# Orange-OpenSource/Cool-Chic

Measured on AMD Instinct MI355X. Metric: decoded Mpixel/s, higher is better.
Workload: dtype int64+f64 entropy / f32 synthesis; 1 GPU; kodak24; frames_on_rank0=24, frame=512x768 RGB 8-bit, HOP decoder

## Files before the change

### cool_chic_amd/csrc/ccd_entropy_pipe.hip

```cpp
#include <hip/hip_runtime.h>
#include <type_traits>

#include "ccd_device.hpp"
#include "ccd_kernels.hpp"
#include "ccd_laplace.hpp"

namespace ccd {

#if defined(CCD_PIPE_PROFILE) && CCD_PIPE_PROFILE >= 3
#define PROF_T() __builtin_amdgcn_s_memtime()
#define PROF_ADD(var, t0) var += __builtin_amdgcn_s_memtime() - (t0)
#define PROF_SUB(var, t0) var -= __builtin_amdgcn_s_memtime() - (t0)
#else
#define PROF_T() 0ull
#define PROF_ADD(var, t0) (void)(t0)
#define PROF_SUB(var, t0) (void)(t0)
#endif
#if defined(CCD_PIPE_PROFILE) && CCD_PIPE_PROFILE == 2 && defined(CCD_PIPE_TRACE)
#define LPROF_T(cond) __builtin_amdgcn_s_memtime()
#elif defined(CCD_PIPE_PROFILE) && CCD_PIPE_PROFILE == 2
#define LPROF_T(cond) ((cond) ? __builtin_amdgcn_s_memtime() : 0ull)
#else
#define LPROF_T(cond) 0ull
#endif
// ... 942 lines not shown
        int64_t acc = C.s_b[(n_layers - 1) * dim + 2 + o];
        const int32_t* w = C.s_w + C.n_w_hidden + 2 * in_pad + o * in_pad;
#pragma unroll 1
        for (int k = 0; k < dim; ++k) acc += static_cast<int64_t>(ain[k]) * w[k];
        stab[o] = acc;
    }
#pragma unroll 1
    for (int l = 0; l < n_layers - 1; ++l) {
#pragma unroll 1
        for (int o = 0; o < dim; ++o) {
            int64_t acc = C.s_b[l * dim + o];
            const int32_t* w = C.s_w + l * dim * in_pad + o * in_pad;
#pragma unroll 1
            for (int k = 0; k < dim; ++k) acc += static_cast<int64_t>(ain[k]) * w[k];
            aout[o] = static_cast<int32_t>((acc < 0 ? 0 : acc) >> 16);
        }
        int32_t* t = ain; ain = aout; aout = t;
    }
#pragma unroll
    for (int o = 0; o < 2; ++o) {
        int64_t acc = C.s_b[(n_layers - 1) * dim + o] + stab[o];
        const int32_t* w = C.s_w + C.n_w_hidden + o * in_pad;
#pragma unroll 1
        for (int k = 0; k < dim; ++k) acc += static_cast<int64_t>(ain[k]) * w[k];
        if (o == 0) out_mu = acc; else out_ls = acc;
    }
}

constexpr int16_t kFeatSentinel = -32768;

struct ExactArgs {
    const EntropyParams* P;
    uint32_t s_w, s_b, s_ring;
    int n_w_hidden, dim, n_layers, n_sp, in_pad;
    int W, fin, fw, feat_plane, ring_mask, fstride;
};
struct ExactOut { int64_t mu, ls; };
__device__ __forceinline__ ExactOut exact_pixel(const ExactArgs& A, int y, int x) {
    const EntropyParams& P = *A.P;
    const int lane = threadIdx.x & 63;
    const int dim = A.dim, n_layers = A.n_layers, n_sp = A.n_sp, in_pad = A.in_pad;
    const int32_t* s_w = reinterpret_cast<const int32_t*>(ccd_pipe_smem + A.s_w);
    const int64_t* s_b = reinterpret_cast<const int64_t*>(ccd_pipe_smem + A.s_b);
    const int8_t* s_ring = reinterpret_cast<const int8_t*>(ccd_pipe_smem + A.s_ring);
    uint64_t xin = 0;
    if (lane < dim) {
        int64_t v = 0;
        if (lane < n_sp) {
            const int yy = y - P.ctx_dy[lane], xx = x + P.ctx_dx[lane];
            if (yy >= 0 && xx >= 0 && xx < A.W) v = s_ring[(yy & A.ring_mask) * 64 + ((xx + 10 * yy) & 63)];
        } else if (A.fin > 0) {
            const int pos = (y >> 1) * A.fw + (x >> 1);
            v = reinterpret_cast<const int16_t*>(P.ifce_feat)[pos * A.fstride + (lane - n_sp)];
            if (v == kFeatSentinel) v = static_cast<int64_t>(static_cast<float>(P.ifce_wide[(lane - n_sp) * A.feat_plane + pos]));
        }
        xin = static_cast<uint64_t>(v) << 16;
    }
    auto bcast = [&](uint64_t v, int k) {
        const uint32_t lo = static_cast<uint32_t>(__shfl(static_cast<int>(static_cast<uint32_t>(v)), k));
        const uint32_t hi = static_cast<uint32_t>(__shfl(static_cast<int>(static_cast<uint32_t>(v >> 32)), k));
        return (static_cast<uint64_t>(hi) << 32) | lo;
    };
    auto layer = [&](const int32_t* wt, const int64_t* bias, int n_out, uint64_t xv) {
        const int o = min(lane, n_out - 1);
        uint64_t acc = static_cast<uint64_t>(bias[o]);
#pragma unroll 1
        for (int k = 0; k < dim; ++k) acc += bcast(xv, k) * static_cast<uint64_t>(static_cast<int64_t>(wt[o * in_pad + k]));
        return acc;
    };
    const uint64_t stab = layer(s_w + A.n_w_hidden + 2 * in_pad, s_b + (n_layers - 1) * dim + 2, 2, xin);
    uint64_t xv = xin;
#pragma unroll 1
    for (int l = 0; l < n_layers - 1; ++l) {
        const int64_t a = static_cast<int64_t>(layer(s_w + l * dim * in_pad, s_b + l * dim, dim, xv));
        xv = static_cast<uint64_t>((a < 0 ? 0 : a) >> 16);
    }
    const uint64_t out = layer(s_w + A.n_w_hidden, s_b + (n_layers - 1) * dim, 2, xv) + stab;
    ExactOut r;
    r.mu = static_cast<int64_t>(bcast(out, 0));
    r.ls = static_cast<int64_t>(bcast(out, 1));
    return r;
}

template <int NV, int kLpp, bool MF, bool DYN_RING, bool DYN, class SH>
__device__ __forceinline__ uint32_t producer_grid(const PipeCtx& C_run, unsigned long long* prof, const GridSeg& seg) {
    constexpr int in_pad = 4 * NV;
    static_assert(!SH::fixed || (!MF && SH::dim <= in_pad && SH::dim > in_pad - 4 && SH::n_sp >= 1 && SH::n_layers >= 2), "ShapeFix: vector-ALU path, matching width");
    PipeCtx C_fix = C_run;
    if constexpr (SH::fixed) {
        constexpr PipeLayout L = pipe_layout(SH::dim, SH::n_layers, in_pad, kRingRows, 0);
        C_fix.s_ring.off = L.ring; C_fix.s_w.off = L.w; C_fix.s_b.off = L.b; C_fix.s_act.off = L.act; C_fix.s_a.off = L.a; C_fix.s_tab.off = L.tab;
        C_fix.s_meta.off = L.meta; C_fix.s_rcp.off = L.rcp; C_fix.s_exp.off = L.exp; C_fix.s_ready.off = L.ready; C_fix.s_consumed.off = L.consumed;
        C_fix.s_abort.off = L.abort; C_fix.n_w_hidden = L.n_w_hidden; C_fix.ring_mask = kRingRows - 1;
#if defined(CCD_PIPE_TRACE)
        C_fix.trace_off = L.end;
#endif
        C_fix.dim = SH::dim; C_fix.n_layers = SH::n_layers; C_fix.n_sp = SH::n_sp; C_fix.k_left = 0;
    }
    const PipeCtx& C = C_fix;
    constexpr int kTaskPix = 64 / kLpp;
    constexpr int kBpx = kTaskPix == 2 ? 8 : 16;
    constexpr int kHalves = kBpx / kTaskPix;
    constexpr int kNSlots = kRows / kBpx;
    constexpr int NOUT = (in_pad + kLpp - 1) / kLpp;
    const int lane = threadIdx.x & 63;
    const int pw = uni(static_cast<int>(threadIdx.x >> 6) - 1);
    const EntropyParams& P = *C.P;
    const int dim = SH::fixed ? SH::dim : uni(C.dim), n_layers = SH::fixed ? SH::n_layers : uni(C.n_layers), n_sp = SH::fixed ? SH::n_sp : uni(C.n_sp);
    const int W = uni(C.W);
    const int k_left = SH::fixed ? 0 : uni(C.k_left), fin = uni(C.fin), fw = uni(C.fw);
    const uint32_t seq_base = uni(C.seq_base);
    int32_t* act = C.s_act + pw * ((DYN_RING ? 16 : 8) * in_pad + 4);
    int32_t* const act_dummy = act + (DYN_RING ? 16 : 8) * in_pad;
    (void)act_dummy;
    const int px = MF ? (lane & 15) : lane / kLpp;
    const int q = MF ? (lane >> 4) : lane % kLpp;
    const int ring_mask = DYN_RING ? uni(C.ring_mask) : kRingRows - 1, n_if = uni(C.n_if), mf_bits = uni(P.mfma);
    (void)n_if; (void)mf_bits;
    const int4* act_row = reinterpret_cast<const int4*>(act + px * in_pad);
    unsigned long long lt_prev_end = 0;
    (void)lt_prev_end;
    int ctx_dy_l[NOUT], ctx_dx_l[NOUT];
#pragma unroll
    for (int t = 0; t < NOUT; ++t) {
        const int k = q + kLpp * t;
        ctx_dy_l[t] = k < n_sp ? P.ctx_dy[k] : 0;
        ctx_dx_l[t] = k < n_sp ? P.ctx_dx[k] : 0;
    }
    const glb_ptr<const int16_t> ifce_feat = (glb_ptr<const int16_t>)reinterpret_cast<const int16_t*>(P.ifce_feat);
    const int feat_plane = uni(C.fh) * fw;
    const int fstride = SH::fixed ? feat_stride(SH::dim - SH::n_sp) : uni(C.fstride);
    int32_t mf_dxy[8], mf_wl[7];
    if constexpr (MF) {
#pragma unroll
        for (int t = 0; t < 8; ++t) {
            const int k = q + 4 * t;
            mf_dxy[t] = k < n_sp ? static_cast<int32_t>((static_cast<uint32_t>(P.ctx_dy[k]) << 16) | (static_cast<uint32_t>(P.ctx_dx[k]) & 0xffffu)) : 0;
        }
#pragma unroll
        for (int r = 0; r < 7; ++r) {
            const int o = r < 4 ? 4 * q + r : 16 + q;
            int32_t w = 0;
            if (k_left >= 0) {
                if (r < 5) w = o < dim ? C.s_w[o * in_pad + k_left] : 0;
                else w = C.s_w[C.n_w_hidden + 2 * in_pad + (r - 5) * in_pad + k_left];
            }
            mf_wl[r] = w;
        }
    }
    (void)mf_dxy; (void)mf_wl;
    constexpr uint32_t kTaskShift = kTaskPix == 8 ? 3 : (kTaskPix == 4 ? 2 : 1), kBpxShift = kBpx == 32 ? 5 : (kBpx == 16 ? 4 : 3), kHalvesShift = kBpxShift - kTaskShift;
    StepWalk it;
    it.init(static_cast<uint32_t>(uni(C.H)), static_cast<uint32_t>(W));
    uint32_t seq = seq_base;
    uint32_t pix0 = uni(C.px_base), prev_pix0 = pix0, prev2_pix0 = pix0, prev_moved = 0;
    const uint32_t seg_first = uni(seg.first), seg_steps = uni(seg.steps);
    const bool seg_body = uni(seg.body ? 1 : 0) != 0;
    if (seg_first > 0u) {
        it.seek_before(seg_first);
        pix0 += uni(seg.pix_before);
        prev_pix0 = pix0 - it.n;
        prev2_pix0 = prev_pix0 - (seg_first > 1u ? it.len_of(seg_first - 2u) : 0u);
        prev_moved = it.moved;
    }
    uint32_t phase = static_cast<uint32_t>((static_cast<unsigned long long>(seq_base) * kHalves) % kProducers);
    const bool split = k_left >= 0 && W > 9 && n_layers >= 2;
    const uint32_t n_steps_total = it.W <= 9u ? it.H * it.W : it.W + 10u * (it.H - 1u);
    const uint32_t seg_end = seg_first + seg_steps;
    const auto walk_on = [&]() {
        prev2_pix0 = prev_pix0; prev_pix0 = pix0; pix0 += it.n; prev_moved = it.moved;
        const uint32_t nx = it.x0 + 1u, mv = nx == it.W ? 1u : 0u;
        it.x0 = mv ? it.W - 10u : nx; it.y0 += mv; it.moved = mv; --it.left;
        it.n = min(it.H - it.y0, ((it.x0 * 0xcccdu) >> 19) + 1u);
    };
    while (n_steps_total - it.left < seg_end && it.next()) {
        const uint32_t seg_n = seg_body ? uni(seg.n_pix) : it.n;
        const uint32_t seg_pix0 = pix0;
        const uint32_t nb = (seg_n + kBpx - 1) >> kBpxShift;
        const uint32_t n_tasks = (seg_n + kTaskPix - 1) >> kTaskShift;
        const uint32_t seq0 = seq;
        uint32_t t_first = static_cast<uint32_t>(pw) - phase;
        t_first += static_cast<int32_t>(t_first) < 0 ? kProducers : 0;
        {
            for (uint32_t task = t_first; task < n_tasks; task += kProducers) {
                const uint32_t j = task >> kHalvesShift;
                const int half = static_cast<int>(task & (kHalves - 1));
                seq = seq0 + j;
                const int slot = static_cast<int>(seq & (kNSlots - 1));
                const int i0 = static_cast<int>(task << kTaskShift);
                const int cnt = min(kTaskPix, static_cast<int>(seg_n) - i0);
                while (seg_pix0 + static_cast<uint32_t>(i0) >= pix0 + it.n) walk_on();
                const uint32_t ia = seg_pix0 + static_cast<uint32_t>(i0) - pix0;
                const uint32_t n_a = min(static_cast<uint32_t>(cnt), it.n - ia);
                const uint32_t bx1 = it.x0 + 1u, b_moved = bx1 == static_cast<uint32_t>(W) ? 1u : 0u;
                const uint32_t bx0 = b_moved ? static_cast<uint32_t>(W) - 10u : bx1, by0 = it.y0 + b_moved;
                const bool in_b = static_cast<uint32_t>(px) >= n_a;
                const int ii = in_b ? px - static_cast<int>(n_a) : static_cast<int>(ia) + px;
                const int y = static_cast<int>(in_b ? by0 : it.y0) + ii, x = static_cast<int>(in_b ? bx0 : it.x0) - 10 * ii;
                const uint32_t dy1 = it.moved, dy2 = it.moved + prev_moved;
                const uint32_t prev_n = pix0 - prev_pix0, prev2_n = prev_pix0 - prev2_pix0;
                uint32_t f_raw[NOUT];
                bool f_has[NOUT];
                if constexpr (!MF) {
                    const int fo = (y >> 1) * fw + (x >> 1);
#pragma unroll
                    for (int t = 0; t < NOUT; ++t) {
                        const int k = q + kLpp * t;
                        f_has[t] = fin > 0 && px < cnt && k >= n_sp && k < dim;
                        f_raw[t] = reinterpret_cast<glb_ptr<const uint16_t>>(ifce_feat)[f_has[t] ? fo * fstride + (k - n_sp) : 0];
                    }
                } else {
#pragma unroll
                    for (int t = 0; t < NOUT; ++t) { f_raw[t] = 0; f_has[t] = false; }
                }
                unsigned long long bad_lanes = 0ull;
                const uint32_t need_slot = seq >= static_cast<uint32_t>(kNSlots) ? seq - kNSlots + 1 : 0;
                const bool ends_in_b = n_a < static_cast<uint32_t>(cnt);
                const uint32_t last1 = ends_in_b ? static_cast<uint32_t>(cnt) - n_a : ia + static_cast<uint32_t>(cnt);
                const uint32_t need_px = ends_in_b ? pix0 + min(last1 + b_moved, it.n) : prev_pix0 + min(last1 + dy1, prev_n);
                const uint32_t need_early_px = ends_in_b ? prev_pix0 + min(last1 + b_moved + dy1, prev_n)
                                                         : prev2_pix0 + min(last1 + dy2, prev2_n);
                unsigned long long lt_a = 0, lt_b = 0, lt_c = 0, lt_d = 0;
                (void)lt_a; (void)lt_b; (void)lt_c; (void)lt_d;
                unsigned narrow_mask = 0;
                constexpr int kPasses = (kTaskPix + 3) / 4;
                uint32_t win_mu[kPasses] = {}, win_rcp[kPasses] = {}, win_ent[kPasses] = {}, win_top[kPasses] = {};
                uint32_t win_left_m = 0, win_keep_m = 0, win_e0 = 0, win_e1 = 0;
                (void)win_mu; (void)win_rcp; (void)win_ent; (void)win_top; (void)win_left_m; (void)win_keep_m; (void)win_e0; (void)win_e1;
                unsigned long long wide_lanes = 0ull;
                RowMeta& meta = *C.s_meta;
                if constexpr (MF) {
                    const int n = px, g = q;
                    const bool live = n < cnt;
                    int32_t f0 = 0, f1 = 0;
                    if (live && fin > 0) {
                        const int fo = (y >> 1) * fw + (x >> 1);
                        if (g < n_if) f0 = ifce_feat[fo * fstride + g];
                        if (g + 4 < n_if) f1 = ifce_feat[fo * fstride + g + 4];
                    }
                    lt_a = LPROF_T(pw == 0);
#if defined(CCD_PIPE_PROFILE) && CCD_PIPE_PROFILE == 2
                    if (pw == 0 && lt_prev_end) prof[4] += lt_a - lt_prev_end;
#endif
                    {
                        const unsigned long long t0 = PROF_T();
                        if (!wait_ge2(C.s_consumed, need_slot, split ? need_early_px : need_px, C.s_abort)) return seq;
                        PROF_ADD(prof[0], t0);
                    }
                    lt_b = LPROF_T(pw == 0);
                    const unsigned long long t_g = PROF_T();
                    {
                        const int mi = (g == 0 && live) ? slot * kBpx + half * kTaskPix + n : kRows;
                        meta.cell[mi] = static_cast<uint32_t>(((y & ring_mask) << 6) | ((x + 10 * y) & 63));
                        meta.goff[mi] = static_cast<uint32_t>(y * W + x);
                    }
                    uint32_t w0 = 0, w1 = 0;
#pragma unroll
                    for (int t = 0; t < 8; ++t) {
                        if (4 * t < n_sp) {
                            const int k = g + 4 * t;
                            const int yy = y - (mf_dxy[t] >> 16), xx = x + static_cast<int16_t>(mf_dxy[t] & 0xffff);
                            const bool take = live && k < n_sp && yy >= 0 && xx >= 0 && xx < W && !(split && k == k_left);
                            const int cell = take ? (yy & ring_mask) * 64 + ((xx + 10 * yy) & 63) : 0;
                            int32_t v = C.s_ring[cell];
                            v = take ? v : 0;
                            if (t < 4) w0 |= static_cast<uint32_t>(v & 0xff) << (8 * t);
                            else w1 |= static_cast<uint32_t>(v & 0xff) << (8 * (t - 4));
                        }
                    }
                    const uint32_t d0 = (static_cast<uint32_t>(f0) + 0x8080u) ^ 0x8080u, d1 = (static_cast<uint32_t>(f1) + 0x8080u) ^ 0x8080u;
                    const i32x4 bop = {static_cast<int>(w0), static_cast<int>(w1), static_cast<int>((d0 & 0xffffu) | (d1 << 16)), 0};
                    PROF_ADD(prof[1], t_g);
                    const unsigned long long t_m = PROF_T();
                    const i32x4* sa = reinterpret_cast<const i32x4*>(static_cast<uint32_t*>(C.s_a)) + lane;
                    const i32x4 zero4 = {0, 0, 0, 0};
                    int64_t pre[5], st0, st1;
                    {
                        i32x4 c1[2][4];
#pragma unroll
                        for (int t = 0; t < 2; ++t)
#pragma unroll
                            for (int s = 0; s < 4; ++s) c1[t][s] = __builtin_amdgcn_mfma_i32_16x16x64_i8(sa[(t * 4 + s) * 64], bop, zero4, 0, 0, 0);
                        const int64_t* bl = C.s_b;
#pragma unroll
                        for (int r = 0; r < 4; ++r) {
                            const int o = 4 * g + r;
                            const int64_t bias = bl[min(o, dim - 1)];
                            pre[r] = mf_comb4(c1[0], r, o < dim ? bias : 0);
                        }
                        {
                            const int64_t bias = bl[min(16 + g, dim - 1)];
                            pre[4] = mf_comb4(c1[1], 0, 16 + g < dim ? bias : 0);
                        }
                        st0 = mf_comb4(c1[1], 1, bl[(n_layers - 1) * dim + 2]);
                        st1 = mf_comb4(c1[1], 2, bl[(n_layers - 1) * dim + 3]);
                    }
                    const i32x4* sl_out = sa + (kMfLayer1 + (n_layers - 2) * kMfHidden) * 64;
                    i32x4 a_h[10], a_o[5];
                    int64_t b_h[5];
                    if (n_layers > 2) {
#pragma unroll
                        for (int s = 0; s < 10; ++s) a_h[s] = sa[(kMfLayer1 + s) * 64];
#pragma unroll
                        for (int r = 0; r < 5; ++r) {
                            const int o = r < 4 ? 4 * g + r : 16 + g;
                            const int64_t bias = C.s_b[dim + min(o, dim - 1)];
                            b_h[r] = o < dim ? bias : 0;
                        }
                    }
#pragma unroll
                    for (int s = 0; s < 5; ++s) a_o[s] = sl_out[s * 64];
// ... 8 lines not shown
                        PROF_SUB(prof[2], t0);
                        PROF_ADD(prof[5], t0);
                        if (live && x >= 1) xleft = static_cast<int32_t>(C.s_ring[(y & ring_mask) * 64 + ((x - 1 + 10 * y) & 63)]) << 16;
                    }
                    lt_d = LPROF_T(pw == 0);
                    const unsigned long long t_h = PROF_T();
                    int32_t av[5];
                    uint32_t big = 0;
#pragma unroll
                    for (int r = 0; r < 5; ++r) {
                        mad64(pre[r], xleft, mf_wl[r]);
                        const int64_t a = pre[r] < 0 ? 0 : pre[r];
                        av[r] = static_cast<int32_t>(a >> 16);
                        big |= static_cast<uint32_t>(av[r]);
                    }
                    mad64(st0, xleft, mf_wl[5]);
                    mad64(st1, xleft, mf_wl[6]);
                    for (int l = 1; l < n_layers - 1; ++l) {
                        const i32x4 b2 = mf_pack15(av);
                        i32x4 c2[5], c2b[5];
#pragma unroll
                        for (int s = 0; s < 5; ++s) c2[s] = __builtin_amdgcn_mfma_i32_16x16x64_i8(a_h[s], b2, zero4, 0, 0, 0);
                        if (dim > 16) {
#pragma unroll
                            for (int s = 0; s < 5; ++s) c2b[s] = __builtin_amdgcn_mfma_i32_16x16x64_i8(a_h[5 + s], b2, zero4, 0, 0, 0);
                        }
#pragma unroll
                        for (int r = 0; r < 4; ++r) {
                            const int64_t a = mf_comb5(c2, r, b_h[r]);
                            av[r] = static_cast<int32_t>((a < 0 ? 0 : a) >> 16);
                            big |= static_cast<uint32_t>(av[r]);
                        }
                        av[4] = 0;
                        if (dim > 16) {
                            const int64_t a = mf_comb5(c2b, 0, b_h[4]);
                            av[4] = static_cast<int32_t>((a < 0 ? 0 : a) >> 16);
                            big |= static_cast<uint32_t>(av[4]);
                        }
                        if (l + 1 < n_layers - 1) {
                            const i32x4* sl = sa + (kMfLayer1 + l * kMfHidden) * 64;
#pragma unroll
                            for (int s = 0; s < 10; ++s) a_h[s] = sl[s * 64];
#pragma unroll
                            for (int r = 0; r < 5; ++r) {
                                const int o = r < 4 ? 4 * g + r : 16 + g;
                                const int64_t bias = C.s_b[(l + 1) * dim + min(o, dim - 1)];
                                b_h[r] = o < dim ? bias : 0;
                            }
                        }
                    }
                    PROF_ADD(prof[6], t_h);
                    const unsigned long long t_o = PROF_T();
                    int64_t out_mu, out_ls;
                    {
                        const i32x4 b3 = mf_pack15(av);
                        i32x4 c3[5];
#pragma unroll
                        for (int s = 0; s < 5; ++s) c3[s] = __builtin_amdgcn_mfma_i32_16x16x64_i8(a_o[s], b3, zero4, 0, 0, 0);
                        out_mu = mf_comb5(c3, 0, b_mu) + st0;
                        out_ls = mf_comb5(c3, 1, b_ls) + st1;
                    }
                    if (__ballot((big >> mf_bits) != 0u) != 0ull) {
                        if (g == 0 && live) mf_exact_task<NV>(C, act, n, y, x, W, fin, fw, feat_plane, ring_mask, out_mu, out_ls);
                    }
                    const int64_t m8 = (out_mu >> 24) + kMuOffset, s8 = (out_ls >> 24) + kScaleOffset;
                    const int32_t idx_mu = static_cast<int32_t>(m8 < 0 ? 0 : (m8 > kNumMu - 1 ? kNumMu - 1 : m8));
                    const int32_t idx_sc = static_cast<int32_t>(s8 < 0 ? 0 : (s8 > kNumScale - 1 ? kNumScale - 1 : s8));
                    const int mpx = slot * kBpx + half * kTaskPix + n;
                    if (g == 0 && live) {
                        meta.mu_idx[mpx] = idx_mu;
                        meta.rcp[mpx] = C.s_rcp[idx_sc];
                    }
                    narrow_mask = static_cast<unsigned>(__ballot(g == 0 && live && idx_sc <= kNarrowMaxScale)) & 0xffffu;
                    PROF_ADD(prof[2], t_m);
                    PROF_ADD(prof[7], t_o);
#if defined(CCD_PIPE_PROFILE) && CCD_PIPE_PROFILE >= 3
                    prof[8] += 1;
#endif
                } else {
                lt_a = LPROF_T(pw == 0);
#if defined(CCD_PIPE_PROFILE) && CCD_PIPE_PROFILE == 2
                if (pw == 0 && lt_prev_end) prof[4] += lt_a - lt_prev_end;
#endif
                {
                    const unsigned long long t0 = PROF_T();
                    if (!wait_ge2(C.s_consumed, need_slot, split ? need_early_px : need_px, C.s_abort)) return seq;
                    PROF_ADD(prof[0], t0);
                }
                lt_b = LPROF_T(pw == 0);
                const unsigned long long t_g = PROF_T();
                {
                    const int mi = (q == 0 && px < cnt) ? slot * kBpx + half * kTaskPix + px : kRows;
                    meta.cell[mi] = static_cast<uint32_t>(((y & ring_mask) << 6) | ((x + 10 * y) & 63));
                    meta.goff[mi] = static_cast<uint32_t>(y * W + x);
                }
                {
                    typedef unsigned int u32x4 __attribute__((ext_vector_type(4)));
                    const u32x4 z4 = {0u, 0u, 0u, 0u};
                    uint2* const tab0 = C.s_tab + static_cast<size_t>(slot * kBpx + half * kTaskPix) * 64;
#pragma unroll
                    for (int j = 0; j < (kTaskPix * 24 + 63) / 64; ++j) {
                        const int t = lane + 64 * j, row = t / 24, e2 = t - 24 * row;
                        uint2* const dst = row < cnt ? &tab0[row * 64 + 16 + 2 * e2] : C.s_tab + kRows * 64 + 16 + 2 * (e2 % 24);
                        *reinterpret_cast<u32x4*>(dst) = z4;
                    }
                }
                {
                    int32_t rr[NOUT];
#pragma unroll
                    for (int t = 0; t < NOUT; ++t) {
                        const int yy = y - ctx_dy_l[t], xx = x + ctx_dx_l[t];
                        rr[t] = C.s_ring[(yy & ring_mask) * 64 + ((xx + 10 * yy) & 63)];
                    }
                    if constexpr (NOUT == 1) asm volatile("" : "+v"(rr[0]));
                    else if constexpr (NOUT == 2) asm volatile("" : "+v"(rr[0]), "+v"(rr[1]));
                    else if constexpr (NOUT == 3) asm volatile("" : "+v"(rr[0]), "+v"(rr[1]), "+v"(rr[2]));
                    else if constexpr (NOUT == 4) asm volatile("" : "+v"(rr[0]), "+v"(rr[1]), "+v"(rr[2]), "+v"(rr[3]));
                    else {
#pragma unroll
                        for (int t = 0; t < NOUT; ++t) asm volatile("" : "+v"(rr[t]));
                    }
                    int32_t fv[NOUT];
                    bool feat_bad = false;
#pragma unroll
                    for (int t = 0; t < NOUT; ++t) {
                        asm volatile("" : "+v"(f_raw[t]));
                        fv[t] = f_has[t] ? static_cast<int32_t>(static_cast<int16_t>(f_raw[t])) : 0;
                        feat_bad |= DYN && fv[t] == kFeatSentinel;
                    }
                    if constexpr (DYN) bad_lanes = __ballot(feat_bad);
#pragma unroll
                    for (int t = 0; t < NOUT; ++t) {
                        const int k = q + kLpp * t;
                        const int yy = y - ctx_dy_l[t], xx = x + ctx_dx_l[t];
                        const int32_t v = k < n_sp ? ((yy >= 0 && xx >= 0 && xx < W && !(split && k == k_left)) ? rr[t] : 0) : fv[t];
                        int32_t* const dst = k < in_pad ? act + px * in_pad + k : act_dummy;
                        *dst = v << 16;
                    }
                }
                PROF_ADD(prof[1], t_g);
                const unsigned long long t_m = PROF_T();
                int4 xv[NV];
#pragma unroll
                for (int v = 0; v < NV; ++v) xv[v] = act_row[v];
                PROF_ADD(prof[4], t_m);
                const unsigned long long t_s = PROF_T();
                int64_t so[2];
                const int qs = q < 2 ? q : 1;
                {
                    const int4* wr = reinterpret_cast<const int4*>(C.s_w + C.n_w_hidden + 2 * in_pad + qs * in_pad);
                    so[0] = C.s_b[(n_layers - 1) * dim + 2 + qs];
                    so[1] = 0;
                    int4 wv[NV];
#pragma unroll
                    for (int v = 0; v < NV; ++v) wv[v] = wr[v];
#pragma unroll
                    for (int v = 0; v < NV; ++v) {
                        const int4 w = wv[v];
                        mad64(so[0], xv[v].x, w.x); mad64(so[1], xv[v].y, w.y); mad64(so[0], xv[v].z, w.z); mad64(so[1], xv[v].w, w.w);
                    }
                }
                PROF_ADD(prof[5], t_s);
                const unsigned long long t_h = PROF_T();
                int64_t acc0[NOUT], acc0_b = 0;
                (void)acc0_b;
                int32_t wleft[NOUT], wleft_stab = 0;
                if (n_layers >= 2) {
                    const int32_t* wl = C.s_w;
                    const int64_t* bl = C.s_b;
                    const int4* wr[NOUT];
                    const int kl = split ? k_left : 0;
#pragma unroll
                    for (int t = 0; t < NOUT; ++t) {
                        const int oc = min(q + kLpp * t, dim - 1);
                        wr[t] = reinterpret_cast<const int4*>(wl + oc * in_pad);
                        acc0[t] = bl[oc];
                        wleft[t] = wl[oc * in_pad + kl];
                    }
                    wleft_stab = C.s_w[C.n_w_hidden + 2 * in_pad + qs * in_pad + kl];
                    int4 w[NOUT], wn[NOUT];
#pragma unroll
                    for (int t = 0; t < NOUT; ++t) w[t] = wr[t][0];
#pragma unroll
                    for (int v = 0; v < NV; ++v) {
                        if (v + 1 < NV) {
#pragma unroll
                            for (int t = 0; t < NOUT; ++t) wn[t] = wr[t][v + 1];
                        }
                        if constexpr (NOUT == 1) { CCD_MAD4_PAIR(acc0, acc0_b, xv[v], w) } else { CCD_MAD4(acc0, xv[v], w, NOUT) }
#pragma unroll
                        for (int t = 0; t < NOUT; ++t) w[t] = wn[t];
                    }
                    if constexpr (NOUT == 1) acc0[0] += acc0_b;
                }
                int32_t xleft = 0;
                const int mpx = slot * kBpx + half * kTaskPix + px;
                uint32_t mu_dst = lds_addr(&meta.mu_idx[px < cnt && q == 0 ? mpx : kRows]);
                uint32_t rcp_dst = lds_addr(&meta.rcp[px < cnt && q == 1 ? mpx : kRows]);
                int32_t rcp_lanes = q == 1 ? -1 : 0, wide_above = px < cnt && q == 1 ? kNarrowMaxScale : 0x7fffffff;
                asm volatile("" : "+v"(mu_dst), "+v"(rcp_dst), "+v"(rcp_lanes), "+v"(wide_above));
#pragma unroll
                for (int k = 0; k < kPasses; ++k) {
                    const int u = lane >> 4, e = lane & 15;
                    const int mine = 4 * k + u;
                    const bool valid = mine < cnt;
                    const int mi = slot * kBpx + half * kTaskPix + (valid ? mine : 4 * k);
                    win_mu[k] = lds_addr(&meta.mu_idx[mi]);
                    win_rcp[k] = lds_addr(&meta.rcp[mi]);
                    win_ent[k] = lds_addr(&C.s_tab[static_cast<size_t>(valid ? mi : kRows) * 64 + e]);
                    win_top[k] = lds_addr(&meta.top[valid && e == 0 ? mi : kRows]);
                    asm volatile("" : "+v"(win_mu[k]), "+v"(win_rcp[k]), "+v"(win_ent[k]), "+v"(win_top[k]));
                }
                win_left_m = (lane & 15) == 15 ? 0u : ~0u;
                win_keep_m = ((lane & 15) == 0 || (lane & 15) == 15) ? 0u : ~0u;
                win_e0 = (lane & 15) == 0 ? (1u << kRcPrecision) - 1u : 0u;
                win_e1 = (lane & 15) == 1 ? 1u : 0u;
                asm volatile("" : "+v"(win_left_m), "+v"(win_keep_m), "+v"(win_e0), "+v"(win_e1));
                lt_c = LPROF_T(pw == 0);
                if (split) {
                    const unsigned long long t0 = PROF_T();
                    const uint32_t want = uni(need_px);
                    const uint32_t cell = static_cast<uint32_t>((y & ring_mask) * 64 + ((x - 1 + 10 * y) & 63));
                    uint32_t seen_v;
                    int32_t r;
                    asm volatile("ds_read_b32 %0, %2 offset:4\n\tds_read_i8 %1, %3\n\ts_waitcnt lgkmcnt(0)"
                                 : "=&v"(seen_v), "=&v"(r) : "v"(C.s_consumed.off), "v"(C.s_ring.off + cell) : "memory");
                    if (__builtin_expect(static_cast<int32_t>(uni(seen_v) - want) < 0, 0)) {
                        unsigned spins = 0;
                        do {
                            if ((++spins & 1023u) == 0) {
                                if (lds_load_acquire(C.s_abort) != 0) return seq;
                                if (spins > kSpinLimit) { lds_write_release(C.s_abort, static_cast<uint32_t>(-CCD_ERR_HIP)); return seq; }
                            }
                            asm volatile("ds_read_b32 %0, %2 offset:4\n\tds_read_i8 %1, %3\n\ts_waitcnt lgkmcnt(0)"
                                         : "=&v"(seen_v), "=&v"(r) : "v"(C.s_consumed.off), "v"(C.s_ring.off + cell) : "memory");
                        } while (static_cast<int32_t>(uni(seen_v) - want) < 0);
                    }
                    PROF_ADD(prof[0], t0);
                    PROF_SUB(prof[2], t0);
                    PROF_SUB(prof[6], t0);
                    xleft = (px < cnt && x >= 1) ? r << 16 : 0;
                }
                lt_d = LPROF_T(pw == 0);
                __builtin_amdgcn_s_setprio(1);
                mad64(so[0], xleft, wleft_stab);
                const int64_t stab = so[0] + so[1];
                if (n_layers >= 2) {
#pragma unroll
                    for (int t = 0; t < NOUT; ++t) {
                        mad64(acc0[t], xleft, wleft[t]);
                        const int o = q + kLpp * t;
                        int32_t* const dst = o < dim ? act + px * in_pad + o : act_dummy;
                        *dst = relu_q16(acc0[t]);
                    }
#pragma unroll
                    for (int v = 0; v < NV; ++v) xv[v] = act_row[v];
                }
                for (int l = 1; l < n_layers - 1; ++l) {
                    const int32_t* wl = C.s_w + l * dim * in_pad;
                    const int64_t* bl = C.s_b + l * dim;
                    int64_t acc[NOUT], acc_b = 0;
                    (void)acc_b;
                    const int4* wr[NOUT];
#pragma unroll
                    for (int t = 0; t < NOUT; ++t) {
                        const int oc = min(q + kLpp * t, dim - 1);
                        wr[t] = reinterpret_cast<const int4*>(wl + oc * in_pad);
                        acc[t] = bl[oc];
                    }
                    int4 w[NOUT], wn[NOUT];
#pragma unroll
                    for (int t = 0; t < NOUT; ++t) w[t] = wr[t][0];
#pragma unroll
                    for (int v = 0; v < NV; ++v) {
                        if (v + 1 < NV) {
#pragma unroll
                            for (int t = 0; t < NOUT; ++t) wn[t] = wr[t][v + 1];
                        }
                        if constexpr (NOUT == 1) { CCD_MAD4_PAIR_SEQ(acc, acc_b, xv[v], w) } else { CCD_MAD4_SEQ(acc, xv[v], w, NOUT) }
#pragma unroll
                        for (int t = 0; t < NOUT; ++t) w[t] = wn[t];
                    }
                    if constexpr (NOUT == 1) acc[0] += acc_b;
#pragma unroll
                    for (int t = 0; t < NOUT; ++t) {
                        const int o = q + kLpp * t;
                        int32_t* const dst = o < dim ? act + px * in_pad + o : act_dummy;
                        *dst = relu_q16(acc[t]);
                    }
#pragma unroll
                    for (int v = 0; v < NV; ++v) xv[v] = act_row[v];
                }
                PROF_ADD(prof[6], t_h);
                const unsigned long long t_o = PROF_T();
                int32_t idx = 0;
                {
                    const int4* wr = reinterpret_cast<const int4*>(C.s_w + C.n_w_hidden + qs * in_pad);
                    int64_t ao[4] = {C.s_b[(n_layers - 1) * dim + qs] + stab, 0, 0, 0};
                    int4 wv[NV];
#pragma unroll
                    for (int v = 0; v < NV; ++v) wv[v] = wr[v];
#pragma unroll
                    for (int v = 0; v < NV; ++v) { CCD_MAD4_QUAD_SEQ(ao, xv[v], wv[v]) }
                    const int64_t acc = (ao[0] + ao[1]) + (ao[2] + ao[3]);
                    const int64_t q8 = acc >> 24;
                    const int64_t off = q8 + (q == 0 ? kMuOffset : kScaleOffset);
                    const int64_t hi = q == 0 ? kNumMu - 1 : kNumScale - 1;
                    idx = static_cast<int32_t>(off < 0 ? 0 : (off > hi ? hi : off));
                    *lds_at<int32_t>(mu_dst) = idx;
                    *lds_at<double>(rcp_dst) = C.s_rcp[idx & rcp_lanes];
                }
                if (DYN && __builtin_expect(bad_lanes != 0ull, 0)) {
                    int n_redo = 0;
                    for (int p = 0; p < cnt; ++p) {
                        if (((bad_lanes >> (p * kLpp)) & ((1ull << kLpp) - 1ull)) == 0ull) continue;
                        ExactArgs A;
                        A.P = C.P; A.s_w = uni(C.s_w.off); A.s_b = uni(C.s_b.off); A.s_ring = uni(C.s_ring.off);
                        A.n_w_hidden = uni(C.n_w_hidden); A.dim = dim; A.n_layers = n_layers; A.n_sp = n_sp; A.in_pad = in_pad;
                        A.W = W; A.fin = fin; A.fw = fw; A.feat_plane = feat_plane; A.ring_mask = ring_mask; A.fstride = fstride;
                        asm volatile("" : "+s"(A.P), "+s"(A.s_w), "+s"(A.s_b), "+s"(A.s_ring), "+s"(A.n_w_hidden), "+s"(A.dim), "+s"(A.n_layers));
                        asm volatile("" : "+s"(A.n_sp), "+s"(A.W), "+s"(A.fin), "+s"(A.fw), "+s"(A.feat_plane), "+s"(A.ring_mask), "+s"(A.fstride));
                        const ExactOut r = exact_pixel(A, __builtin_amdgcn_readlane(y, MF ? p : p * kLpp), __builtin_amdgcn_readlane(x, MF ? p : p * kLpp));
                        if (px == p && q < 2) {
                            const int64_t off = ((q == 0 ? r.mu : r.ls) >> 24) + (q == 0 ? kMuOffset : kScaleOffset);
                            const int64_t hi = q == 0 ? kNumMu - 1 : kNumScale - 1;
                            idx = static_cast<int32_t>(off < 0 ? 0 : (off > hi ? hi : off));
                            if (q == 0) {
                                meta.mu_idx[mpx] = idx;
                            } else {
                                    meta.rcp[mpx] = C.s_rcp[idx];
                            }
                        }
                        ++n_redo;
                    }
                    if (lane == 0) atomicAdd(reinterpret_cast<int*>(P.status) + 39, n_redo);
                }
                wide_lanes = __ballot(idx > wide_above);
                PROF_ADD(prof[2], t_m);
                PROF_ADD(prof[7], t_o);
#if defined(CCD_PIPE_PROFILE) && CCD_PIPE_PROFILE >= 3
                prof[8] += 1;
#endif
                }
                const unsigned long long t_t = PROF_T();
                const int base = slot * kBpx + half * kTaskPix;
                uint2* tab = C.s_tab + static_cast<size_t>(base) * 64;
                if constexpr (!MF) {
#pragma unroll
                    for (int k = 0; k < kPasses; ++k) {
                        if (k > 0 && 4 * k >= cnt) break;
                        const int e = lane & 15;
                        const int mu_idx = *lds_at<int32_t>(win_mu[k]);
                        const double rcp256 = window_rcp256(*lds_at<double>(win_rcp[k]));
                        int top = ((mu_idx + 128) >> 8) - 64 + 6;
                        top = max(kAcLo + 13, min(kAcLo + kAlphabet - 1, top));
                        const int ssym = top - (e - 1);
                        const uint32_t lo_m = static_cast<uint32_t>((kAcLo - ssym) >> 31) & win_left_m;
                        const bool at_top = top == kAcLo + kAlphabet - 1;
                        const uint32_t hi_f = at_top ? win_e0 : 0u, to_full = at_top ? win_e1 : 0u;
                        uint32_t left = window_cum_d256(window_d256(mu_idx, ssym), rcp256, C.s_exp) + static_cast<uint32_t>(ssym - kAcLo);
                        left = (min(left, (1u << kRcPrecision) - 1u) | hi_f) & lo_m;
                        const uint32_t right = static_cast<uint32_t>(__builtin_amdgcn_update_dpp(0, static_cast<int>(left), 0x111, 0xf, 0xf, false));
                        uint2 ent;
                        ent.x = left;
                        ent.y = (right - left + to_full) & win_keep_m;
                        typedef unsigned int u32x2 __attribute__((ext_vector_type(2)));
                        const u32x2 ent2 = {ent.x, ent.y};
                        *lds_at<u32x2>(win_ent[k]) = ent2;
                        *lds_at<int32_t>(win_top[k]) = top;
                    }
                }
                unsigned rest = MF ? narrow_mask : 0u;
                while (rest) {
                    int pix[4];
                    int n_here = 0;
#pragma unroll
                    for (int u = 0; u < 4; ++u) {
                        pix[u] = rest ? __builtin_ctz(rest) : -1;
                        if (rest) { rest &= rest - 1; ++n_here; }
                    }
                    const int u = lane >> 4, e = lane & 15;
                    const int mine = u == 0 ? pix[0] : (u == 1 ? pix[1] : (u == 2 ? pix[2] : pix[3]));
                    const int mi = base + (mine < 0 ? pix[0] : mine);
                    const int mu_idx = meta.mu_idx[mi];
                    int top = ((mu_idx + 128) >> 8) - 64 + 6;
                    top = max(kAcLo + 13, min(kAcLo + kAlphabet - 1, top));
                    const double mu = -64.0 + static_cast<double>(mu_idx) * (1.0 / 256.0);
                    const int ssym = top - (e - 1);
                    uint32_t left = min(window_left(mu, meta.rcp[mi], ssym, C.s_exp), (1u << kRcPrecision) - 1u);
                    left = e == 15 ? 0u : left;
                    const uint32_t right = static_cast<uint32_t>(__builtin_amdgcn_update_dpp(0, static_cast<int>(left), 0x111, 0xf, 0xf, false));
                    uint2 ent;
                    ent.x = left;
                    ent.y = (e == 0 || e == 15) ? 0u : ((e == 1 && ssym == kAcLo + kAlphabet - 1) ? (1u << kRcPrecision) - left : right - left);
                    if (mine >= 0) {
                        tab[mine * 64 + e] = ent;
                        if (e == 0) meta.top[mi] = top;
                    }
                    if constexpr (MF) {
                        typedef unsigned int u32x4 __attribute__((ext_vector_type(4)));
                        const u32x4 z4 = {0u, 0u, 0u, 0u};
#pragma unroll
                        for (int j = 0; j < 2; ++j) {
                            const int t = lane + 64 * j;
                            const int ru = t >= 72 ? 3 : (t >= 48 ? 2 : (t >= 24 ? 1 : 0));
                            const int rp = ru == 0 ? pix[0] : (ru == 1 ? pix[1] : (ru == 2 ? pix[2] : pix[3]));
                            if (t < 96 && rp >= 0) *reinterpret_cast<u32x4*>(&tab[rp * 64 + 16 + 2 * (t - 24 * ru)]) = z4;
                        }
                    }
                    (void)n_here;
                }
                unsigned long long wide = MF ? static_cast<unsigned long long>(((1u << cnt) - 1u) & ~narrow_mask) : wide_lanes;
                while (wide) {
                    const int bit = __builtin_ctzll(wide);
                    wide &= wide - 1;
                    const int i = MF ? bit : bit / kLpp;
                    const int mi = base + i;
                    const int mu_idx = meta.mu_idx[mi];
                    int top = ((mu_idx + 128) >> 8) - 64 + 30;
                    top = max(kAcLo + 61, min(kAcLo + kAlphabet - 1, top));
                    const int ssym = top - (lane - 1);
                    uint32_t left = min(window_left_d256(window_d256(mu_idx, ssym), window_rcp256(meta.rcp[mi]), ssym, C.s_exp), (1u << kRcPrecision) - 1u);
                    left = lane == 63 ? 0u : left;
                    const uint32_t right = __shfl_up(left, 1);
                    uint2 ent;
                    ent.x = left;
                    ent.y = (lane == 0 || lane == 63) ? 0u
                            : ((lane == 1 && ssym == kAcLo + kAlphabet - 1) ? (1u << kRcPrecision) - left : right - left);
                    tab[i * 64 + lane] = ent;
                    if (lane == 0) meta.top[mi] = top;
                }
                asm volatile("" ::: "memory");
                if (lane == 0) __hip_atomic_fetch_or(&C.s_ready[slot], 1u << half, __ATOMIC_RELAXED, __HIP_MEMORY_SCOPE_WORKGROUP);
                __builtin_amdgcn_s_setprio(0);
                asm volatile("" ::: "memory");
                PROF_ADD(prof[3], t_t);
#if defined(CCD_PIPE_PROFILE) && CCD_PIPE_PROFILE == 2
#if defined(CCD_PIPE_TRACE)
                {
                    const unsigned long long lt_e = __builtin_amdgcn_s_memtime();
                    const uint32_t gidx = seq0 * kHalves + task;
                    if (lane == 0 && static_cast<uint32_t>(W) == uni(g_trace_cfg[0]) && uni(g_trace_cfg[1]) - it.left < 64u) {
                        typedef unsigned int u32x4 __attribute__((ext_vector_type(4)));
                                                u32x4* r = reinterpret_cast<u32x4*>(ccd_pipe_smem + C.trace_off + (gidx % kTraceTasks) * 32u);
                        const u32x4 r0 = {(it.left << 12) | ((task & 15u) << 8) | (static_cast<uint32_t>(pw) << 4) | static_cast<uint32_t>(cnt), static_cast<uint32_t>(lt_a),
                                          static_cast<uint32_t>(lt_b), static_cast<uint32_t>(lt_c)};
                        const u32x4 r1 = {static_cast<uint32_t>(lt_d), static_cast<uint32_t>(lt_e), need_px - pix0, static_cast<uint32_t>(lt_a >> 32)};
                        r[0] = r0; r[1] = r1;
                    }
                }
#endif
                if (pw == 0) {
                    const unsigned long long lt_e = __builtin_amdgcn_s_memtime();
                    prof[0] += lt_b - lt_a; prof[1] += lt_c - lt_b; prof[2] += lt_d - lt_c; prof[3] += lt_e - lt_d; prof[8] += 1;
                    lt_prev_end = lt_e;
                }
#endif
            }
        }
        seq = seq0 + nb;
        phase = (phase + nb * kHalves) % kProducers;
        if (seg_body) {
            while (n_steps_total - it.left < seg_end) walk_on();
        }
        prev2_pix0 = prev_pix0;
        prev_pix0 = pix0;
        pix0 += it.n;
        prev_moved = it.moved;
    }
    return seq;
}

template <int NV, bool MF, bool DYN, class SH>
__global__ __launch_bounds__(kPipeThreads) void entropy_pipe_kernel(const EntropyParams* slots_desc) {
    const EntropyParams& P = slots_desc[blockIdx.x];
    const int tid = threadIdx.x;
    const int lane = tid & 63;
    const int wave = __builtin_amdgcn_readfirstlane(tid >> 6);
    const int dim = P.dim;
    constexpr int in_pad = 4 * NV;
    const int n_layers = P.n_layers;
    const int n_if = P.has_ifce ? P.n_ifce_out : 0;

    PipeCtx C;
    C.P = &P;
    const int ring_rows = MF ? P.ring_rows : kRingRows;
    {
        const PipeLayout L = pipe_layout(dim, n_layers, in_pad, ring_rows, MF ? mf_tables(n_layers) : 0);
        C.s_ring.off = L.ring; C.s_w.off = L.w; C.s_b.off = L.b; C.s_act.off = L.act; C.s_a.off = L.a; C.s_tab.off = L.tab;
        C.s_meta.off = L.meta; C.s_rcp.off = L.rcp; C.s_exp.off = L.exp; C.s_ready.off = L.ready; C.s_consumed.off = L.consumed;
        C.s_abort.off = L.abort; C.n_w_hidden = L.n_w_hidden;
#if defined(CCD_PIPE_TRACE)
        C.trace_off = L.end;
#endif
    }
    C.ring_mask = ring_rows - 1;
    constexpr int kActRows = MF ? 16 : 8;
    double* s_rcp = smem_at<double>(C.s_rcp.off);
    double* s_exp = smem_at<double>(C.s_exp.off);
    for (int i = tid; i < kNumScale; i += kPipeThreads) s_rcp[i] = P.rcp_table[i];
    for (int i = tid; i < kExpN; i += kPipeThreads) s_exp[i] = kExpTab[i];
    C.dim = dim; C.n_layers = n_layers; C.n_sp = P.n_spatial; C.n_if = n_if;
    C.fstride = feat_stride(n_if);
    C.k_left = -1;
    for (int k = 0; k < P.n_spatial; ++k) if (P.ctx_dy[k] == 0 && P.ctx_dx[k] == -1) C.k_left = k;

    {
        const int64_t* src = P.arm;
        for (int l = 0; l < n_layers; ++l) {
            const int n_out = (l == n_layers - 1) ? 2 : dim;
            int32_t* wt = C.s_w + (l < n_layers - 1 ? l * dim * in_pad : C.n_w_hidden);
            for (int i = tid; i < n_out * in_pad; i += kPipeThreads) {
                const int o = i / in_pad, k = i - o * in_pad;
                wt[i] = k < dim ? static_cast<int32_t>(src[k * n_out + o]) : 0;
            }
            int64_t* bb = C.s_b + (l < n_layers - 1 ? l * dim : (n_layers - 1) * dim);
// ... 371 lines not shown
```

Baseline: 265.4 Mpixel/s.

## Fuse output layer into per-lane partial sums with DPP reduction and per-pixel table build

The entropy producer's last MLP layer no longer writes the final hidden activations to LDS and re-reads a full row per output lane. Each lane now multiplies its own hidden outputs by the output weights and the partial sums are combined with 64-bit DPP lane reductions. The window/probability table is built by each pixel's own lane group instead of in extra cross-pixel passes that re-read mu/rcp from LDS. The ready-flag atomic is issued through inline asm with exec forced to a single lane. This cuts LDS round-trips and serial passes, but adds fragile DPP/exec inline assembly and depends on specific RowMeta layout assumptions.

```diff
diff --git a/cool_chic_amd/csrc/ccd_entropy_pipe.hip b/cool_chic_amd/csrc/ccd_entropy_pipe.hip
--- a/cool_chic_amd/csrc/ccd_entropy_pipe.hip
+++ b/cool_chic_amd/csrc/ccd_entropy_pipe.hip
@@ -1048,6 +1048,38 @@
     return r;
 }
 
+template <int CTRL>
+__device__ __forceinline__ int64_t dpp_add64(int64_t v) {
+    const uint32_t lo = static_cast<uint32_t>(__builtin_amdgcn_mov_dpp(static_cast<int>(v), CTRL, 0xf, 0xf, true));
+    const uint32_t hi = static_cast<uint32_t>(__builtin_amdgcn_mov_dpp(static_cast<int>(v >> 32), CTRL, 0xf, 0xf, true));
+    typedef unsigned int u32x2 __attribute__((ext_vector_type(2)));
+    const u32x2 other = {lo, hi};
+    return v + __builtin_bit_cast(int64_t, other);
+}
+__device__ __forceinline__ int64_t dpp_add64_row_below(int64_t v) {
+    const uint32_t lo = static_cast<uint32_t>(__builtin_amdgcn_update_dpp(0, static_cast<int>(v), 0x142, 0xa, 0xf, false));
+    const uint32_t hi = static_cast<uint32_t>(__builtin_amdgcn_update_dpp(0, static_cast<int>(v >> 32), 0x142, 0xa, 0xf, false));
+    typedef unsigned int u32x2 __attribute__((ext_vector_type(2)));
+    const u32x2 other = {lo, hi};
+    return v + __builtin_bit_cast(int64_t, other);
+}
+template <int LANES>
+__device__ __forceinline__ void group_sum2(int64_t& a, int64_t& b) {
+    static_assert(LANES == 8 || LANES == 16 || LANES == 32, "a pixel's lane group: part of a DPP row, a row, or two rows");
+    a = dpp_add64<0xB1>(a); b = dpp_add64<0xB1>(b);
+    a = dpp_add64<0x4E>(a); b = dpp_add64<0x4E>(b);
+    a = dpp_add64<0x141>(a); b = dpp_add64<0x141>(b);
+    if constexpr (LANES >= 16) { a = dpp_add64<0x140>(a); b = dpp_add64<0x140>(b); }
+    if constexpr (LANES == 32) { a = dpp_add64_row_below(a); b = dpp_add64_row_below(b); }
+}
+__device__ __forceinline__ int32_t table_index(int64_t sum, int32_t off, int32_t hi) {
+    const int32_t h = min(max(static_cast<int32_t>(sum >> 32), -(1 << 22)), 1 << 22);
+    const int32_t x = static_cast<int32_t>((static_cast<uint32_t>(h) << 8) | (static_cast<uint32_t>(sum) >> 24));
+    return min(max(x + off, 0), hi);
+}
+static_assert(kMuOffset < (1 << 29) && kScaleOffset < (1 << 29) && kMuOffset >= 0 && kScaleOffset >= 0, "table_index: offsets");
+static_assert(offsetof(RowMeta, top) - offsetof(RowMeta, mu_idx) == (kRows + 2) * 4, "a pixel's top symbol is stored (kRows + 2) words behind its mu index");
+
 template <int NV, int kLpp, bool MF, bool DYN_RING, bool DYN, class SH>
 __device__ __forceinline__ uint32_t producer_grid(const PipeCtx& C_run, unsigned long long* prof, const GridSeg& seg) {
     constexpr int in_pad = 4 * NV;
@@ -1189,10 +1221,18 @@
                 unsigned long long lt_a = 0, lt_b = 0, lt_c = 0, lt_d = 0;
                 (void)lt_a; (void)lt_b; (void)lt_c; (void)lt_d;
                 unsigned narrow_mask = 0;
-                constexpr int kPasses = (kTaskPix + 3) / 4;
-                uint32_t win_mu[kPasses] = {}, win_rcp[kPasses] = {}, win_ent[kPasses] = {}, win_top[kPasses] = {};
                 uint32_t win_left_m = 0, win_keep_m = 0, win_e0 = 0, win_e1 = 0;
-                (void)win_mu; (void)win_rcp; (void)win_ent; (void)win_top; (void)win_left_m; (void)win_keep_m; (void)win_e0; (void)win_e1;
+                (void)win_left_m; (void)win_keep_m; (void)win_e0; (void)win_e1;
+                constexpr int kQ0 = kLpp == 32 ? 16 : 0;
+                constexpr int kEpl = kLpp == 8 ? 2 : 1;
+                const int e0 = kEpl * (q & 15);
+                int32_t idx_mu = 0, idx_sc = 0;
+                double own_rcp = 0.0;
+                uint32_t own_ent = 0;
+                uint32_t mu_dst = 0, rcp_dst = 0;
+                (void)idx_mu; (void)idx_sc; (void)own_rcp; (void)own_ent; (void)mu_dst; (void)rcp_dst;
+                uint32_t rdy_addr = 0, rdy_val = 0;
+                (void)rdy_addr; (void)rdy_val;
                 unsigned long long wide_lanes = 0ull;
                 RowMeta& meta = *C.s_meta;
                 if constexpr (MF) {
@@ -1367,6 +1407,7 @@
 #if defined(CCD_PIPE_PROFILE) && CCD_PIPE_PROFILE == 2
                 if (pw == 0 && lt_prev_end) prof[4] += lt_a - lt_prev_end;
 #endif
+                int32_t hid[NOUT];
                 {
                     const unsigned long long t0 = PROF_T();
                     if (!wait_ge2(C.s_consumed, need_slot, split ? need_early_px : need_px, C.s_abort)) return seq;
@@ -1421,6 +1462,7 @@
                         const int32_t v = k < n_sp ? ((yy >= 0 && xx >= 0 && xx < W && !(split && k == k_left)) ? rr[t] : 0) : fv[t];
                         int32_t* const dst = k < in_pad ? act + px * in_pad + k : act_dummy;
                         *dst = v << 16;
+                        hid[t] = v << 16;
                     }
                 }
                 PROF_ADD(prof[1], t_g);
@@ -1479,28 +1521,44 @@
                     if constexpr (NOUT == 1) acc0[0] += acc0_b;
                 }
                 int32_t xleft = 0;
+                int qo = q;
+                asm volatile("" : "+v"(qo));
                 const int mpx = slot * kBpx + half * kTaskPix + px;
-                uint32_t mu_dst = lds_addr(&meta.mu_idx[px < cnt && q == 0 ? mpx : kRows]);
-                uint32_t rcp_dst = lds_addr(&meta.rcp[px < cnt && q == 1 ? mpx : kRows]);
-                int32_t rcp_lanes = q == 1 ? -1 : 0, wide_above = px < cnt && q == 1 ? kNarrowMaxScale : 0x7fffffff;
-                asm volatile("" : "+v"(mu_dst), "+v"(rcp_dst), "+v"(rcp_lanes), "+v"(wide_above));
-#pragma unroll
-                for (int k = 0; k < kPasses; ++k) {
-                    const int u = lane >> 4, e = lane & 15;
-                    const int mine = 4 * k + u;
-                    const bool valid = mine < cnt;
-                    const int mi = slot * kBpx + half * kTaskPix + (valid ? mine : 4 * k);
-                    win_mu[k] = lds_addr(&meta.mu_idx[mi]);
-                    win_rcp[k] = lds_addr(&meta.rcp[mi]);
-                    win_ent[k] = lds_addr(&C.s_tab[static_cast<size_t>(valid ? mi : kRows) * 64 + e]);
-                    win_top[k] = lds_addr(&meta.top[valid && e == 0 ? mi : kRows]);
-                    asm volatile("" : "+v"(win_mu[k]), "+v"(win_rcp[k]), "+v"(win_ent[k]), "+v"(win_top[k]));
+                mu_dst = lds_addr(&meta.mu_idx[px < cnt && qo == kQ0 ? mpx : kRows]);
+                rcp_dst = lds_addr(&meta.rcp[px < cnt && qo == kQ0 + 1 ? mpx : kRows]);
+                int32_t wide_above = px < cnt && qo == kQ0 + 1 ? kNarrowMaxScale : 0x7fffffff;
+                asm volatile("" : "+v"(mu_dst), "+v"(rcp_dst), "+v"(wide_above));
+                int64_t out_m = 0, out_l = 0;
+                int32_t wl_m = 0, wl_l = 0, wo_m[NOUT], wo_l[NOUT];
+                (void)wl_m; (void)wl_l; (void)wo_m; (void)wo_l;
+                {
+                    const int64_t s = so[0] + so[1] + C.s_b[(n_layers - 1) * dim + qs];
+                    const int64_t keep_m = qo == 0 ? -1 : 0, keep_l = qo == 1 ? -1 : 0;
+                    out_m = s & keep_m;
+                    out_l = s & keep_l;
+                    wl_m = wleft_stab & static_cast<int32_t>(keep_m);
+                    wl_l = wleft_stab & static_cast<int32_t>(keep_l);
+                    asm volatile("" : "+v"(out_m), "+v"(out_l), "+v"(wl_m), "+v"(wl_l));
+                    const int32_t* const w_out = C.s_w + C.n_w_hidden;
+#pragma unroll
+                    for (int t = 0; t < NOUT; ++t) {
+                        const int o = qo + kLpp * t, oc = min(o, in_pad - 1);
+                        const int32_t keep = (o - dim) >> 31;
+                        wo_m[t] = w_out[oc] & keep;
+                        wo_l[t] = w_out[in_pad + oc] & keep;
+                        asm volatile("" : "+v"(wo_m[t]), "+v"(wo_l[t]));
+                    }
                 }
-                win_left_m = (lane & 15) == 15 ? 0u : ~0u;
-                win_keep_m = ((lane & 15) == 0 || (lane & 15) == 15) ? 0u : ~0u;
-                win_e0 = (lane & 15) == 0 ? (1u << kRcPrecision) - 1u : 0u;
-                win_e1 = (lane & 15) == 1 ? 1u : 0u;
-                asm volatile("" : "+v"(win_left_m), "+v"(win_keep_m), "+v"(win_e0), "+v"(win_e1));
+                rdy_addr = lds_addr(&C.s_ready[slot]);
+                rdy_val = 1u << half;
+                asm volatile("" : "+v"(rdy_addr), "+v"(rdy_val));
+                const int e0o = kEpl * (qo & 15);
+                own_ent = lds_addr(&C.s_tab[static_cast<size_t>(px < cnt && qo >= kQ0 ? mpx : kRows) * 64 + e0o]);
+                win_left_m = e0o + kEpl - 1 == 15 ? 0u : ~0u;
+                win_keep_m = (e0o == 0 || e0o == 15) ? 0u : ~0u;
+                win_e0 = e0o == 0 ? (1u << kRcPrecision) - 1u : 0u;
+                win_e1 = (e0o <= 1 && e0o + kEpl > 1) ? 1u : 0u;
+                asm volatile("" : "+v"(own_ent), "+v"(win_left_m), "+v"(win_keep_m), "+v"(win_e0), "+v"(win_e1));
                 lt_c = LPROF_T(pw == 0);
                 if (split) {
                     const unsigned long long t0 = PROF_T();
@@ -1528,18 +1586,24 @@
                 }
                 lt_d = LPROF_T(pw == 0);
                 __builtin_amdgcn_s_setprio(1);
-                mad64(so[0], xleft, wleft_stab);
-                const int64_t stab = so[0] + so[1];
+                mad64(out_m, xleft, wl_m);
+                mad64(out_l, xleft, wl_l);
                 if (n_layers >= 2) {
 #pragma unroll
                     for (int t = 0; t < NOUT; ++t) {
                         mad64(acc0[t], xleft, wleft[t]);
-                        const int o = q + kLpp * t;
-                        int32_t* const dst = o < dim ? act + px * in_pad + o : act_dummy;
-                        *dst = relu_q16(acc0[t]);
-                    }
-#pragma unroll
-                    for (int v = 0; v < NV; ++v) xv[v] = act_row[v];
+                        hid[t] = relu_q16(acc0[t]);
+                    }
+                    if (n_layers > 2) {
+#pragma unroll
+                        for (int t = 0; t < NOUT; ++t) {
+                            const int o = q + kLpp * t;
+                            int32_t* const dst = o < dim ? act + px * in_pad + o : act_dummy;
+                            *dst = hid[t];
+                        }
+#pragma unroll
+                        for (int v = 0; v < NV; ++v) xv[v] = act_row[v];
+                    }
                 }
                 for (int l = 1; l < n_layers - 1; ++l) {
                     const int32_t* wl = C.s_w + l * dim * in_pad;
@@ -1569,32 +1633,28 @@
                     if constexpr (NOUT == 1) acc[0] += acc_b;
 #pragma unroll
                     for (int t = 0; t < NOUT; ++t) {
-                        const int o = q + kLpp * t;
-                        int32_t* const dst = o < dim ? act + px * in_pad + o : act_dummy;
-                        *dst = relu_q16(acc[t]);
-                    }
-#pragma unroll
-                    for (int v = 0; v < NV; ++v) xv[v] = act_row[v];
+                        hid[t] = relu_q16(acc[t]);
+                        asm("" : "+v"(hid[t]));
+                    }
+                    if (l + 2 < n_layers) {
+#pragma unroll
+                        for (int t = 0; t < NOUT; ++t) {
+                            const int o = q + kLpp * t;
+                            int32_t* const dst = o < dim ? act + px * in_pad + o : act_dummy;
+                            *dst = hid[t];
+                        }
+#pragma unroll
+                        for (int v = 0; v < NV; ++v) xv[v] = act_row[v];
+                    }
                 }
                 PROF_ADD(prof[6], t_h);
                 const unsigned long long t_o = PROF_T();
-                int32_t idx = 0;
-                {
-                    const int4* wr = reinterpret_cast<const int4*>(C.s_w + C.n_w_hidden + qs * in_pad);
-                    int64_t ao[4] = {C.s_b[(n_layers - 1) * dim + qs] + stab, 0, 0, 0};
-                    int4 wv[NV];
-#pragma unroll
-                    for (int v = 0; v < NV; ++v) wv[v] = wr[v];
-#pragma unroll
-                    for (int v = 0; v < NV; ++v) { CCD_MAD4_QUAD_SEQ(ao, xv[v], wv[v]) }
-                    const int64_t acc = (ao[0] + ao[1]) + (ao[2] + ao[3]);
-                    const int64_t q8 = acc >> 24;
-                    const int64_t off = q8 + (q == 0 ? kMuOffset : kScaleOffset);
-                    const int64_t hi = q == 0 ? kNumMu - 1 : kNumScale - 1;
-                    idx = static_cast<int32_t>(off < 0 ? 0 : (off > hi ? hi : off));
-                    *lds_at<int32_t>(mu_dst) = idx;
-                    *lds_at<double>(rcp_dst) = C.s_rcp[idx & rcp_lanes];
-                }
+#pragma unroll
+                for (int t = 0; t < NOUT; ++t) { mad64_seq(out_m, hid[t], wo_m[t]); mad64_seq(out_l, hid[t], wo_l[t]); }
+                group_sum2<kLpp>(out_m, out_l);
+                idx_mu = table_index(out_m, kMuOffset, kNumMu - 1);
+                idx_sc = table_index(out_l, kScaleOffset, kNumScale - 1);
+                own_rcp = C.s_rcp[idx_sc];
                 if (DYN && __builtin_expect(bad_lanes != 0ull, 0)) {
                     int n_redo = 0;
                     for (int p = 0; p < cnt; ++p) {
@@ -1606,21 +1666,16 @@
                         asm volatile("" : "+s"(A.P), "+s"(A.s_w), "+s"(A.s_b), "+s"(A.s_ring), "+s"(A.n_w_hidden), "+s"(A.dim), "+s"(A.n_layers));
                         asm volatile("" : "+s"(A.n_sp), "+s"(A.W), "+s"(A.fin), "+s"(A.fw), "+s"(A.feat_plane), "+s"(A.ring_mask), "+s"(A.fstride));
                         const ExactOut r = exact_pixel(A, __builtin_amdgcn_readlane(y, MF ? p : p * kLpp), __builtin_amdgcn_readlane(x, MF ? p : p * kLpp));
-                        if (px == p && q < 2) {
-                            const int64_t off = ((q == 0 ? r.mu : r.ls) >> 24) + (q == 0 ? kMuOffset : kScaleOffset);
-                            const int64_t hi = q == 0 ? kNumMu - 1 : kNumScale - 1;
-                            idx = static_cast<int32_t>(off < 0 ? 0 : (off > hi ? hi : off));
-                            if (q == 0) {
-                                meta.mu_idx[mpx] = idx;
-                            } else {
-                                    meta.rcp[mpx] = C.s_rcp[idx];
-                            }
+                        if (px == p) {
+                            idx_mu = table_index(r.mu, kMuOffset, kNumMu - 1);
+                            idx_sc = table_index(r.ls, kScaleOffset, kNumScale - 1);
+                            own_rcp = C.s_rcp[idx_sc];
                         }
                         ++n_redo;
                     }
                     if (lane == 0) atomicAdd(reinterpret_cast<int*>(P.status) + 39, n_redo);
                 }
-                wide_lanes = __ballot(idx > wide_above);
+                wide_lanes = __ballot(idx_sc > wide_above);
                 PROF_ADD(prof[2], t_m);
                 PROF_ADD(prof[7], t_o);
 #if defined(CCD_PIPE_PROFILE) && CCD_PIPE_PROFILE >= 3
@@ -1631,28 +1686,37 @@
                 const int base = slot * kBpx + half * kTaskPix;
                 uint2* tab = C.s_tab + static_cast<size_t>(base) * 64;
                 if constexpr (!MF) {
-#pragma unroll
-                    for (int k = 0; k < kPasses; ++k) {
-                        if (k > 0 && 4 * k >= cnt) break;
-                        const int e = lane & 15;
-                        const int mu_idx = *lds_at<int32_t>(win_mu[k]);
-                        const double rcp256 = window_rcp256(*lds_at<double>(win_rcp[k]));
-                        int top = ((mu_idx + 128) >> 8) - 64 + 6;
+                    {
+                        int top = ((idx_mu + 128) >> 8) - 64 + 6;
                         top = max(kAcLo + 13, min(kAcLo + kAlphabet - 1, top));
-                        const int ssym = top - (e - 1);
-                        const uint32_t lo_m = static_cast<uint32_t>((kAcLo - ssym) >> 31) & win_left_m;
+                        lds_at<int32_t>(mu_dst)[0] = idx_mu;
+                        lds_at<int32_t>(mu_dst)[kRows + 2] = top;
+                        const double rcp256 = window_rcp256(own_rcp);
+                        *lds_at<double>(rcp_dst) = own_rcp;
                         const bool at_top = top == kAcLo + kAlphabet - 1;
                         const uint32_t hi_f = at_top ? win_e0 : 0u, to_full = at_top ? win_e1 : 0u;
-                        uint32_t left = window_cum_d256(window_d256(mu_idx, ssym), rcp256, C.s_exp) + static_cast<uint32_t>(ssym - kAcLo);
-                        left = (min(left, (1u << kRcPrecision) - 1u) | hi_f) & lo_m;
-                        const uint32_t right = static_cast<uint32_t>(__builtin_amdgcn_update_dpp(0, static_cast<int>(left), 0x111, 0xf, 0xf, false));
-                        uint2 ent;
-                        ent.x = left;
-                        ent.y = (right - left + to_full) & win_keep_m;
-                        typedef unsigned int u32x2 __attribute__((ext_vector_type(2)));
-                        const u32x2 ent2 = {ent.x, ent.y};
-                        *lds_at<u32x2>(win_ent[k]) = ent2;
-                        *lds_at<int32_t>(win_top[k]) = top;
+                        uint32_t left[kEpl];
+#pragma unroll
+                        for (int j = 0; j < kEpl; ++j) {
+                            const int ssym = top - (e0 + j - 1);
+                            uint32_t lo_m = static_cast<uint32_t>((kAcLo - ssym) >> 31);
+                            if (j == kEpl - 1) lo_m &= win_left_m;
+                            uint32_t l = window_cum_d256(window_d256(idx_mu, ssym), rcp256, C.s_exp) + static_cast<uint32_t>(ssym - kAcLo);
+                            l = min(l, (1u << kRcPrecision) - 1u);
+                            if (j == 0) l |= hi_f;
+                            left[j] = l & lo_m;
+                            if (j + 1 < kEpl) __builtin_amdgcn_sched_barrier(0);
+                        }
+                        const uint32_t right = static_cast<uint32_t>(__builtin_amdgcn_update_dpp(0, static_cast<int>(left[kEpl - 1]), 0x111, 0xf, 0xf, false));
+                        if constexpr (kEpl == 1) {
+                            typedef unsigned int u32x2 __attribute__((ext_vector_type(2)));
+                            const u32x2 ent = {left[0], (right - left[0] + to_full) & win_keep_m};
+                            *lds_at<u32x2>(own_ent) = ent;
+                        } else {
+                            typedef unsigned int u32x4 __attribute__((ext_vector_type(4)));
+                            const u32x4 ent = {left[0], (right - left[0]) & win_keep_m, left[1], (left[0] - left[1] + to_full) & win_left_m};
+                            *lds_at<u32x4>(own_ent) = ent;
+                        }
                     }
                 }
                 unsigned rest = MF ? narrow_mask : 0u;
@@ -1716,7 +1780,13 @@
                     if (lane == 0) meta.top[mi] = top;
                 }
                 asm volatile("" ::: "memory");
-                if (lane == 0) __hip_atomic_fetch_or(&C.s_ready[slot], 1u << half, __ATOMIC_RELAXED, __HIP_MEMORY_SCOPE_WORKGROUP);
+                if constexpr (!MF) {
+                    unsigned long long exec_all;
+                    asm volatile("s_mov_b64 %0, exec\n\ts_mov_b64 exec, 1\n\tds_or_b32 %1, %2\n\ts_mov_b64 exec, %0"
+                                 : "=&s"(exec_all) : "v"(rdy_addr), "v"(rdy_val) : "memory");
+                } else {
+                    if (lane == 0) __hip_atomic_fetch_or(&C.s_ready[slot], 1u << half, __ATOMIC_RELAXED, __HIP_MEMORY_SCOPE_WORKGROUP);
+                }
                 __builtin_amdgcn_s_setprio(0);
                 asm volatile("" ::: "memory");
                 PROF_ADD(prof[3], t_t);
```

Result: faster. 274.3 Mpixel/s (median of 6 runs) (+3.3%).
